# roeiherz/CanonicalSg2Im

Hardware: AMD Instinct MI355X
Metric: 256x256 images/sec/node (G+D step) (higher is better)
Workload: dtype f32; 1 GPU; BASELINE config C3: COCO-shaped AttSPADE 256x256, batch 16/GPU, 1-30 objects/img, ngf=64 ndf=64, --no_vgg_loss --use_img_disc 0; Sg2Layout GCN + SPADE G + 2-scale PatchGAN D + object-crop D, fwd+bwd+Adam; global_batch=16, parallelism=dp1

## Files before the change

### canonicalsg2im_amd/_lib.py

```python
import ctypes
import os

import torch

_HERE = os.path.dirname(os.path.abspath(__file__))
LIB_PATH = os.environ.get("CSG_HIP_LIB") or os.path.join(_HERE, "libcsg_hip.so")

MAX_TAPS = 16
ACT_NONE, ACT_LEAKY, ACT_TANH = 0, 1, 2

c_i32, c_i64, c_f32, c_f64, c_p = ctypes.c_int32, ctypes.c_int64, ctypes.c_float, ctypes.c_double, ctypes.c_void_p


class ConvDesc(ctypes.Structure):
    _fields_ = [
        ("B", c_i32), ("IHp", c_i32), ("IWp", c_i32), ("Cin", c_i32), ("x_cs", c_i32),
        ("IHv", c_i32), ("IWv", c_i32), ("in_up", c_i32),
        ("OHg", c_i32), ("OWg", c_i32), ("OHf", c_i32), ("OWf", c_i32), ("os", c_i32), ("ooy", c_i32), ("oox", c_i32),
        ("Cout", c_i32), ("y_cs", c_i32),
        ("istride", c_i32), ("ntaps", c_i32), ("wtaps", c_i32),
        ("tap_dy", c_i32 * MAX_TAPS), ("tap_dx", c_i32 * MAX_TAPS), ("tap_w", c_i32 * MAX_TAPS),
        ("act", c_i32), ("slope", c_f32), ("accumulate", c_i32), ("res_gate", c_i32),
    ]

# ... 68 lines not shown
    "csg_layout_bwd": (c_i32, [c_p, c_i64, c_i64, c_p, c_p, c_p, c_i64, c_i64, c_i64, c_i64, c_i64, c_i64, c_i64,
                               c_i64, c_p, c_i32, c_p, c_p, c_p, c_i64, c_p]),
    "csg_layout_bwd_masks": (c_i32, [c_p, c_i64, c_i64, c_p, c_p, c_i64, c_i64, c_i64, c_i64, c_i64, c_i64, c_i64, c_i64,
                                     c_p, c_p, c_i32, c_p]),
    "csg_layout_mass": (c_i32, [c_p, c_p, c_p, c_p, c_i64, c_i64, c_i64, c_i64, c_i64, c_i64, c_p, c_p]),
    "csg_layout_paint": (c_i32, [c_p, c_p, c_p, c_i64, c_p, c_i64, c_i64, c_i64, c_i64, c_i64, c_i64, c_i64, c_p, c_i64,
                                 c_i64, c_p]),
    "csg_conv_fwd_workspace": (c_i64, [ctypes.POINTER(ConvDesc)]),
    "csg_conv_fwd": (c_i32, [ctypes.POINTER(ConvDesc), c_p, c_p, c_p, c_p, c_p, c_p, c_i64, c_p]),
    "csg_conv_bwd_weight_workspace": (c_i64, [ctypes.POINTER(ConvDesc)]),
    "csg_conv_bwd_weight": (c_i32, [ctypes.POINTER(ConvDesc), c_p, c_p, c_p, c_p, c_p, c_i64, c_p]),
    "csg_wino_pack_bytes": (c_i64, [c_i64, c_i64]),
    "csg_wino_pack_weights": (c_i32, [c_p, c_i64, c_i64, c_i64, c_i64, c_i64, c_i64, c_i32, c_p, c_p, c_p]),
    "csg_conv_fwd_multi_workspace": (c_i64, [ctypes.POINTER(ConvDesc), c_i32]),
    "csg_conv_fwd_multi": (c_i32, [ctypes.POINTER(ConvDesc), c_i32, c_p, c_p, c_p, c_p, c_p, c_p, c_i64, c_p]),
    "csg_gemm_supported": (c_i32, [ctypes.POINTER(GemmDesc)]),
    "csg_gemm_nt": (c_i32, [ctypes.POINTER(GemmDesc), c_p, c_p, c_p, c_p, c_p, c_p]),
    "csg_gemm_tn_workspace": (c_i64, [c_i64, c_i64, c_i64]),
    "csg_gemm_tn": (c_i32, [c_i64, c_i64, c_i64, c_p, c_i64, c_p, c_i64, c_p, c_p, c_p, c_i64, c_p]),
    "csg_conv_few_supported": (c_i32, [ctypes.POINTER(FewDesc)]),
    "csg_conv_few_fwd_workspace": (c_i64, [ctypes.POINTER(FewDesc)]),
    "csg_conv_few_fwd": (c_i32, [ctypes.POINTER(FewDesc), c_p, c_p, c_p, c_p, c_p, c_i64, c_p]),
    "csg_conv_few_bwd_data": (c_i32, [ctypes.POINTER(FewDesc), c_p, c_p, c_p, c_p]),
    "csg_conv_few_bwd_weight_workspace": (c_i64, [ctypes.POINTER(FewDesc)]),
    "csg_conv_few_bwd_weight": (c_i32, [ctypes.POINTER(FewDesc), c_p, c_p, c_p, c_p, c_p, c_i64, c_p]),
    "csg_wino_conv_workspace": (c_i64, [ctypes.POINTER(WinoDesc)]),
    "csg_wino_conv": (c_i32, [ctypes.POINTER(WinoDesc), c_p, c_p, c_p, c_p, c_p, c_f32, c_p, c_p, c_i64, c_p]),
    "csg_wino_bwd_weight_workspace": (c_i64, [ctypes.POINTER(WinoDesc)]),
    "csg_wino_bwd_weight": (c_i32, [ctypes.POINTER(WinoDesc), c_p, c_p, c_p, c_p, c_p, c_i64, c_p]),
    "csg_wino4_bwd_weight_workspace": (c_i64, [ctypes.POINTER(WinoDesc)]),
    "csg_wino4_bwd_weight": (c_i32, [ctypes.POINTER(WinoDesc), c_p, c_p, c_p, c_p, c_p, c_i64, c_p]),
    "csg_wino4_supported": (c_i32, [ctypes.POINTER(WinoDesc)]),
    "csg_wino4_persistent": (c_i32, [c_i32]),
    "csg_wino_pack_weights_multi": (c_i32, [ctypes.POINTER(WinoPackItem), c_i32, c_p]),
    "csg_wino4_pack_bytes": (c_i64, [c_i64, c_i64]),
    "csg_wino4_pack_weights": (c_i32, [c_p, c_i64, c_i64, c_i64, c_i64, c_i64, c_i64, c_i32, c_p, c_p, c_p]),
    "csg_wino4_conv_workspace": (c_i64, [ctypes.POINTER(WinoDesc)]),
    "csg_wino4_conv": (c_i32, [ctypes.POINTER(WinoDesc), c_p, c_p, c_p, c_p, c_p, c_f32, c_p, c_p, c_i64, c_p]),
    "csg_wino4_conv_part": (c_i32, [ctypes.POINTER(WinoDesc), c_p, c_p, c_i64, c_i64, c_p, c_p, c_p, c_i64, c_p, c_p, c_f32,
                                    c_p, c_p]),
    "csg_wino4_conv_spade_supported": (c_i32, [ctypes.POINTER(WinoDesc)]),
    "csg_wino4_conv_spade": (c_i32, [ctypes.POINTER(WinoDesc), c_p, c_p, c_p, c_p, c_p, c_i64, c_p, c_p, c_f32, c_p, c_p]),
    "csg_wino34_supported": (c_i32, [ctypes.POINTER(WinoDesc), c_i32]),
    "csg_wino34_pack_weights": (c_i32, [c_p, c_i64, c_i64, c_i64, c_i64, c_i64, c_i64, c_i32, c_p, c_p, c_p]),
    "csg_wino34_conv_workspace": (c_i64, [ctypes.POINTER(WinoDesc), c_i32]),
    "csg_wino34_conv": (c_i32, [ctypes.POINTER(WinoDesc), c_i32, c_p, c_p, c_p, c_p, c_p, c_f32, c_p, c_p, c_i64, c_p]),
    "csg_act_bwd": (c_i32, [c_p, c_p, c_i64, c_i32, c_f32, c_p, c_p]),
    "csg_colsum": (c_i32, [c_p, c_i64, c_i64, c_i64, c_p, c_p, c_i64, c_p]),
    "csg_norm_stats": (c_i32, [c_p, c_i64, c_i64, c_i64, c_p, c_p, c_i64, c_p]),
    "csg_norm_finalize": (c_i32, [c_p, c_i64, c_i64, c_f64, c_f32, c_i32, c_p, c_p, c_p, c_p, c_f32, c_p]),
    "csg_norm_stats_finalize": (c_i32, [c_p, c_i64, c_i64, c_i64, c_p, c_i64, c_f64, c_f32, c_p, c_p, c_p, c_p, c_p, c_p, c_f32,
                                        c_p]),
    "csg_norm_apply_fwd": (c_i32, [c_p, c_p, c_p, c_p, c_f32, c_i64, c_i64, c_i64, c_p, c_p, c_f32, c_p, c_p]),
    "csg_norm_eval_stats_multi": (c_i32, [ctypes.POINTER(NormEvalItem), c_i32, c_f32, c_p, c_p]),
    "csg_deprocess_u8_workspace": (c_i64, [c_i64]),
    "csg_deprocess_u8": (c_i32, [c_p, c_i64, c_i64, c_i64, c_i64, ctypes.POINTER(c_f32), ctypes.POINTER(c_f32), c_i32, c_p, c_p,
                                 c_i64, c_p]),
    "csg_preprocess_workspace": (c_i64, [c_p, c_i64, c_i64]),
    "csg_preprocess": (c_i32, [c_p, c_i64, c_p, c_p, c_i64, c_i64, c_i64, ctypes.POINTER(c_f32), ctypes.POINTER(c_f32), c_p, c_p,
                               c_p, c_i64, c_p]),
    "csg_preprocess_px_workspace": (c_i64, [c_p, c_i64, c_i64]),
    "csg_preprocess_px": (c_i32, [c_p, c_i64, c_p, c_p, c_i64, c_i64, c_i64, ctypes.POINTER(c_f32), ctypes.POINTER(c_f32), c_p,
                                  c_p, c_p, c_i64, c_p]),
    "csg_clevr_boxes": (c_i32, [c_p, c_p, c_i64, c_p, c_p, c_p, c_p, c_i64, c_i64, c_p, c_p]),
    "csg_vg_rows": (c_i32, [c_p, c_p, c_p, c_p, c_p, c_p, c_i64, c_i64, c_i64, c_p, c_p, c_p]),
    "csg_draw_boxes_u8": (c_i32, [c_p, c_p, c_p, c_i64, c_i64, c_i64, c_i64, c_i64, c_i64, c_p, c_i64, c_i32, c_p, c_p]),
# ... 108 lines not shown
```

### canonicalsg2im_amd/csrc/wino4.hip

```cpp
#include <stddef.h>
#include <stdlib.h>

#include <type_traits>

#include "csg_buffer.h"
#include "csg_common.h"
#include "csg_pack.h"
#include "csg_reduce.h"

using namespace csg;

typedef __attribute__((ext_vector_type(16))) float f32x16;
typedef const volatile __attribute__((address_space(3))) csg_f32x2* w4_lds_cv2;

#define W4_TW 8
#define W4_TH 4
#define W4_CQ 9
#define W4_PS 8
#define W4_RSE 36
#define W4_NLD 2
#define W4_THREADS 768
#define W4_RBUF (6 * 2 * 32 * W4_RSE)

struct Wino4Params {
// ... 258 lines not shown
          bl2[r] = w4_out_row(2 * half + r, lo) + csg_f32x2{bbv.x, bbv.y};
          bh2[r] = w4_out_row(2 * half + r, hi) + csg_f32x2{bbv.z, bbv.w};
        }
      }
      const float4 mm = *(const float4*)(p.mod_mean + n), mr = *(const float4*)(p.mod_invstd + n);
      const int64_t rowstride = (int64_t)p.Wo * p.y_cs;
      const int64_t pix0 = ((int64_t)img * p.Ho + oy + 2 * half) * p.Wo + ox;
      const int64_t off = pix0 * p.y_cs + n;
      float4 mx[2];
#pragma unroll
      for (int r = 0; r < 2; ++r) mx[r] = *(const float4*)(xin + off + r * rowstride);
#pragma unroll
      for (int r = 0; r < 2; ++r) {
        const csg_f32x2 gl = gl2[r], gh = gh2[r], bl = bl2[r], bh = bh2[r];
        const float gs[4] = {gl.x, gl.y, gh.x, gh.y}, vv[4] = {bl.x, bl.y, bh.x, bh.y};
        const float xs[4] = {mx[r].x, mx[r].y, mx[r].z, mx[r].w};
        const float ms[4] = {mm.x, mm.y, mm.z, mm.w}, rs[4] = {mr.x, mr.y, mr.z, mr.w};
        float out[4];
#pragma unroll
        for (int e = 0; e < 4; ++e) {
          const float xh = (xs[e] - ms[e]) * rs[e];
          float o = xh * (1.f + gs[e]) + vv[e];
          if (p.mod_slope != 1.0f) o = o > 0.f ? o : o * p.mod_slope;
          out[e] = o;
        }
        if (gout != nullptr)
          *(float4*)(gout + (pix0 + (int64_t)r * p.Wo) * p.g_cs + n) = make_float4(gs[0], gs[1], gs[2], gs[3]);
        *(float4*)(y + off + r * rowstride) = make_float4(out[0], out[1], out[2], out[3]);
      }
    }
  }
}

template <int NB>
__device__ __forceinline__ void w4_epilogue(f32x16 (&acc)[6], const Wino4Params& p, float* rbase, int tid, int wave, int grp,
                                            int j, int h, int nt32, int img, int X0, int Y0, const float* __restrict__ bias,
                                            const float* __restrict__ res, const float* __restrict__ gate,
                                            float* __restrict__ y) {
  float* rbuf = rbase + grp * (W4_RBUF / 2 * NB);
  const int tig = tid - grp * (W4_THREADS / 2);
  const bool plain = p.act == CSG_ACT_NONE && res == nullptr && gate == nullptr;
  if (NB == 2) __syncthreads();
  csg_f32x2 rr[NB == 1 ? 4 : 1][8];
  if (NB == 1) {
#pragma unroll
    for (int ge = 0; ge < 8; ++ge) {
#define W4_M(K) csg_f32x2{acc[K][2 * ge], acc[K][2 * ge + 1]}
      const csg_f32x2 m0 = W4_M(0), m1 = W4_M(1), m2 = W4_M(2), m3 = W4_M(3), m4 = W4_M(4), m5 = W4_M(5);
#undef W4_M
      rr[0][ge] = ((m0 + m1) + (m2 + m3)) + m4;
      rr[NB == 1 ? 1 : 0][ge] = w4_pfma(-2.0f, m4, w4_pfma(0.5f, m3, m1 - m2));
      rr[NB == 1 ? 2 : 0][ge] = w4_pfma(4.0f, m4, w4_pfma(0.25f, m3, m1 + m2));
      rr[NB == 1 ? 3 : 0][ge] = w4_pfma(-8.0f, m4, w4_pfma(0.125f, m3, m1 - m2)) + m5;
    }
#pragma unroll
    for (int b = 0; b < (NB == 1 ? 4 : 1); ++b)
#pragma unroll
      for (int ge = 0; ge < 8; ++ge) asm volatile("" : "+v"(rr[b][ge]));
  }
#pragma unroll
  for (int round = 0; round < 4 / NB; ++round) {
#pragma unroll
    for (int g = 0; g < 4; ++g) {
      csg_f32x2 r0[2], r1[2];
#pragma unroll
      for (int e = 0; e < 2; ++e) {
        if (NB == 1) {
          r0[e] = rr[NB == 1 ? round : 0][2 * g + e];
          continue;
        }
#define W4_M(K) csg_f32x2{acc[K][4 * g + 2 * e], acc[K][4 * g + 2 * e + 1]}
        const csg_f32x2 m0 = W4_M(0), m1 = W4_M(1), m2 = W4_M(2), m3 = W4_M(3), m4 = W4_M(4), m5 = W4_M(5);
#undef W4_M
        const int b0 = NB * round;
        if (b0 == 0) r0[e] = ((m0 + m1) + (m2 + m3)) + m4;
        if (b0 == 2) r0[e] = w4_pfma(4.0f, m4, w4_pfma(0.25f, m3, m1 + m2));
        if (b0 == 0) r1[e] = w4_pfma(-2.0f, m4, w4_pfma(0.5f, m3, m1 - m2));
        if (b0 == 2) r1[e] = w4_pfma(-8.0f, m4, w4_pfma(0.125f, m3, m1 - m2)) + m5;
      }
      const int ch = 8 * g + 4 * h;
      *(float4*)(rbuf + ((wave * NB + 0) * 32 + j) * W4_RSE + ch) = make_float4(r0[0].x, r0[0].y, r0[1].x, r0[1].y);
      if (NB == 2)
        *(float4*)(rbuf + ((wave * NB + 1) * 32 + j) * W4_RSE + ch) = make_float4(r1[0].x, r1[0].y, r1[1].x, r1[1].y);
    }
    __syncthreads();
    if (NB == 1 && p.mod == 2)
      w4_store_joint<NB>(p, rbase, tid, round, nt32 - grp * p.gb_off, img, X0, Y0, bias, res, const_cast<float*>(gate), y);
    else if (p.mod)
      w4_store_columns<2, NB>(p, rbuf, tig, round, nt32, img, X0, Y0, bias, res, gate, y);
    else if (plain)
      w4_store_columns<0, NB>(p, rbuf, tig, round, nt32, img, X0, Y0, bias, res, gate, y);
    else
      w4_store_columns<1, NB>(p, rbuf, tig, round, nt32, img, X0, Y0, bias, res, gate, y);
    if (round + 1 < 4 / NB) __syncthreads();
  }
}

__device__ __forceinline__ void w3_epilogue(f32x16 (&acc)[6], const Wino4Params& p, float* smem, int tid, int wave, int grp,
                                            int j, int h, int nt32, int img, int X0, int Y0, const float* __restrict__ bias,
                                            const float* __restrict__ res, const float* __restrict__ gate,
                                            float* __restrict__ y) {
  float* rbuf = smem + grp * W4_RBUF;
  const int tig = tid - grp * (W4_THREADS / 2);
  __syncthreads();
#pragma unroll
  for (int round = 0; round < 2; ++round) {
#pragma unroll
    for (int g = 0; g < 4; ++g) {
      csg_f32x2 r0[2], r1[2];
#pragma unroll
      for (int e = 0; e < 2; ++e) {
#define W4_M(K) csg_f32x2{acc[K][4 * g + 2 * e], acc[K][4 * g + 2 * e + 1]}
        const csg_f32x2 m0 = W4_M(0), m1 = W4_M(1), m2 = W4_M(2), m3 = W4_M(3), m4 = W4_M(4), m5 = W4_M(5);
#undef W4_M
        if (round == 0) {
          r0[e] = ((m0 + m1) + (m2 + m3)) + m4;
          r1[e] = w4_pfma(-2.0f, m4, w4_pfma(0.5f, m3, m1 - m2));
        } else {
          r0[e] = w4_pfma(4.0f, m4, w4_pfma(0.25f, m3, m1 + m2)) + m5;
// ... 60 lines not shown
            vv[0] *= gv.x > 0.f ? 1.f : p.gate_slope; vv[1] *= gv.y > 0.f ? 1.f : p.gate_slope;
            vv[2] *= gv.z > 0.f ? 1.f : p.gate_slope; vv[3] *= gv.w > 0.f ? 1.f : p.gate_slope;
          }
          *(float4*)(y + off) = make_float4(vv[0], vv[1], vv[2], vv[3]);
        }
      }
    }
    if (round == 0) __syncthreads();
  }
}

#define W4_VBUF (36 * 2 * 32 * 4)
template <int T>
struct W4Geo {
  static constexpr int R = T * W4_TH + 6 - T;
  static constexpr int C = T * W4_TW + 6 - T;
  static constexpr int RS = T == 4 ? 288 : 256;
  static constexpr int BUFW = R * RS + 8 + 16;
  static constexpr int V0 = 2 * BUFW;
  static constexpr int OFFTAB = (2 * BUFW + 2 * W4_VBUF) > 2 * W4_RBUF ? (2 * BUFW + 2 * W4_VBUF) : 2 * W4_RBUF;
  static_assert((T * RS) % 64 == 0 && R * C * 2 <= W4_NLD * W4_THREADS && (C + T - 1) / T <= W4_CQ && BUFW < 65536, "staging geometry");
};
#define W4V_RAW0 0
struct W4KernArgs {
  Wino4Params p;
  const float* x;
  const float4* up;
  const float* bias;
  const float* res;
  const float* gate;
  float* y;
};
typedef const __attribute__((address_space(4))) W4KernArgs* w4_kernargs_ptr;
template <int T, bool P>
__global__ __launch_bounds__(W4_THREADS, 3) void k_wino4_conv_v(Wino4Params p, const float* __restrict__ x,
                                                                 const float4* __restrict__ up,
                                                                 const float* __restrict__ bias,
                                                                 const float* __restrict__ res,
                                                                 const float* __restrict__ gate, float* __restrict__ y) {
  typedef W4Geo<T> Geo;
  constexpr int W4_RS = Geo::RS, W4_BUFW = Geo::BUFW, W4V_V0 = Geo::V0, W4V_OFFTAB = Geo::OFFTAB;
  static_assert(!P || T == 4, "the persistent form serves F(4x4,3x3)");
  extern __shared__ __attribute__((aligned(16))) float smem[];
  const int tid = threadIdx.x, lane = tid & 63;
  const int wave12 = __builtin_amdgcn_readfirstlane(tid >> 6);
  const int grp = wave12 >= 6 ? 1 : 0;
  const int wave = wave12 - 6 * grp;

  int nb, img, X0, Y0, split = 0;
  auto decode = [&](int item) {
    if (!P) {
      split = item % p.ksplit;
      item /= p.ksplit;
    }
    nb = item % p.nblocks;
    item /= p.nblocks;
    const int bx = item % p.tbx;
    item /= p.tbx;
    const int by = item % p.tby;
    img = item / p.tby;
    X0 = bx * T * W4_TW;
    Y0 = by * T * W4_TH;
  };
  int v = 0, v_hi = 0, v_step = 1;
  if (P) {
    const int q = p.nitems >> 3, r = p.nitems & 7, xcd = blockIdx.x & 7;
    const int v_lo = xcd < r ? xcd * (q + 1) : r * (q + 1) + (xcd - r) * q;
    v_hi = v_lo + q + (xcd < r ? 1 : 0);
    v_step = gridDim.x >> 3;
    v = v_lo + (blockIdx.x >> 3);
    if (v >= v_hi) return;
    decode(v);
  } else {
    decode(w4_xcd_remap(blockIdx.x, gridDim.x));
  }
// ... 22 lines not shown
          goff[i] = (unsigned)(((img * p.H + iy) * p.W + ix) * p.x_cs + c4 * 4) * 4u;
      }
      loffp |= (unsigned)lo << (16 * i);
    }
    *(uint4*)tab = make_uint4(goff[0], goff[1], loffp, 0u);
  };
  fill_plan(W4_TAB(0), true);
  const int s_begin = split * p.sps, s_end = min(p.nstage, s_begin + p.sps);
  csg_f32x4 st[W4_NLD];
  auto load_stage = [&](int s) {
    const bool over = P && s >= s_end;
    const uint2 go = *(const uint2*)W4_TAB(over ? tsel ^ 1 : tsel);
    if (over) s -= s_end;
    st[0] = csg_buf_load_x4(rsX, (int)go.x, s * (W4_PS * 4), 0);
    st[1] = csg_buf_load_x4(rsX, (int)go.y, s * (W4_PS * 4), 0);
  };
  auto store_stage = [&](float* base) {
    const unsigned lp = s_tab[2];
#pragma unroll
    for (int i = 0; i < W4_NLD; ++i) {
      const unsigned lo = (i & 1) ? (lp >> 16) : (lp & 0xffffu);
      float* dst = base + lo;
      *(float2*)dst = make_float2(st[i].x, st[i].y);
      *(float2*)(dst + 2) = make_float2(st[i].z, st[i].w);
    }
  };

  const int j = lane & 31, h = lane >> 5;
  const int tx = j & (W4_TW - 1), ty = j >> 3;
  const int rb = wave == 0 ? 0 : 1;
  const float* p0 = smem + W4V_RAW0 + (T * ty + rb) * W4_RS + 2 * ty + tx * W4_PS + 4 * grp + 2 * h;
  float* pv = smem + W4V_V0 + (((wave * 6) * 2 + h) * 32 + j) * 4;

  int nt32 = p.gb_off ? nb + grp * p.gb_off : nb * 2 + grp;
  auto u_tile = [&]() { return ((wave * 6) * p.NT32 + nt32 + p.nt_off) * p.Q8 * 1024; };
  const unsigned ulane = nt32 + p.nt_off < p.NT32 || P ? (unsigned)lane * 16u : CSG_OOB_OFF;
  int ubase = u_tile(), ubase_nxt = ubase;
  const int ustride = p.NT32 * p.Q8 * 1024;
  csg_f32x4 ur[3];
  auto load_ur = [&](int slot, int nu, int s) {
    const bool over = P && s >= s_end;
    const int qq = over ? 0 : min(s, p.Q8 - 1);
    ur[slot] = csg_buf_load_x4(rsU, (int)ulane, (over ? ubase_nxt : ubase) + nu * ustride + qq * 1024, 0);
  };

  f32x16 acc[6];

  auto produce_xi = [&](auto xi_tag, int rbufsel, int vbufsel) {
    constexpr int XI = decltype(xi_tag)::value;
    constexpr int RBC = XI == 0 ? 0 : 1;
    constexpr int O2 = 2 * W4_RS + (T == 3 ? 2 * RBC : 0), O3 = 3 * W4_RS + (T == 3 ? 2 : 2 * RBC);
    csg_f32x2 t[6];
#pragma unroll
    for (int c = 0; c < 6; ++c) {
      const int co = rbufsel * W4_BUFW + ((c % T) * W4_CQ + (c / T)) * W4_PS;
      const csg_f32x2 e0 = *(w4_lds_cv2)(p0 + co);
      const csg_f32x2 e1 = *(w4_lds_cv2)(p0 + co + W4_RS);
      const csg_f32x2 e2 = *(w4_lds_cv2)(p0 + co + O2);
      const csg_f32x2 e3 = *(w4_lds_cv2)(p0 + co + O3);
      if (XI == 0 || XI == 5) {
        const csg_f32x2 e4 = *(w4_lds_cv2)(p0 + co + 4 * W4_RS + 2);
        t[c] = w4_pfma(1.5f, e3 - e1, w4_pfma(-2.0f, e2, e0 + e4));
      } else if (XI == 1) {
        t[c] = w4_pfma(2.5f, e2, w4_pfma(0.5f, e1, e3 - e0));
      } else if (XI == 2) {
        t[c] = w4_pfma(0.5f, e2, w4_pfma(-2.5f, e1, e3 + e0));
      } else if (XI == 3) {
        t[c] = w4_pfma(2.0f, e2 - e0, e3 - e1);
      } else {
        t[c] = w4_pfma(-0.5f, e2 - e0, e3 - e1);
      }
    }
    csg_f32x2 v[6];
    {
      const csg_f32x2 s42 = t[4] - t[2], s31 = t[3] - t[1];
      v[0] = w4_pfma(1.5f, s31, w4_pfma(-2.0f, t[2], t[0] + t[4]));
      v[1] = w4_pfma(2.5f, t[3], w4_pfma(0.5f, t[2], t[4] - t[1]));
      v[2] = w4_pfma(0.5f, t[3], w4_pfma(-2.5f, t[2], t[4] + t[1]));
      v[3] = w4_pfma(2.0f, s31, s42);
      v[4] = w4_pfma(-0.5f, s31, s42);
      v[5] = w4_pfma(1.5f, s42, w4_pfma(-2.0f, t[3], t[1] + t[5]));
    }
    int goff2 = 2 * grp;
    if (P) {
      int z;
      asm volatile("s_mov_b32 %0, 0" : "=s"(z));
      goff2 += z;
    }
#pragma unroll
    for (int nu = 0; nu < 6; ++nu)
      *(csg_f32x2*)(pv + vbufsel * W4_VBUF + nu * 256 + goff2) = v[nu];
  };
  auto produce = [&](int rbufsel, int vbufsel) {
    switch (wave) {
      case 0: produce_xi(std::integral_constant<int, 0>(), rbufsel, vbufsel); break;
      case 1: produce_xi(std::integral_constant<int, 1>(), rbufsel, vbufsel); break;
      case 2: produce_xi(std::integral_constant<int, 2>(), rbufsel, vbufsel); break;
      case 3: produce_xi(std::integral_constant<int, 3>(), rbufsel, vbufsel); break;
      case 4: produce_xi(std::integral_constant<int, 4>(), rbufsel, vbufsel); break;
      default: produce_xi(std::integral_constant<int, 5>(), rbufsel, vbufsel); break;
    }
  };
  auto consume = [&](auto lo_tag, auto hi_tag, int vbufsel, int s) {
#pragma unroll
    for (int nu = decltype(lo_tag)::value; nu < decltype(hi_tag)::value; ++nu) {
      const float4 v = *(const float4*)(pv + vbufsel * W4_VBUF + nu * 256);
      const int slot = nu % 3;
      acc[nu] = __builtin_amdgcn_mfma_f32_32x32x2f32(ur[slot].x, v.x, acc[nu], 0, 0, 0);
      acc[nu] = __builtin_amdgcn_mfma_f32_32x32x2f32(ur[slot].y, v.y, acc[nu], 0, 0, 0);
      acc[nu] = __builtin_amdgcn_mfma_f32_32x32x2f32(ur[slot].z, v.z, acc[nu], 0, 0, 0);
      acc[nu] = __builtin_amdgcn_mfma_f32_32x32x2f32(ur[slot].w, v.w, acc[nu], 0, 0, 0);
      if (nu < 3) load_ur(slot, nu + 3, s); else load_ur(slot, nu - 3, s + 1);
    }
  };
  constexpr int SPLIT = 3;
  auto stage = [&](int s, auto par_tag) {
    constexpr int par = decltype(par_tag)::value;
    typedef std::integral_constant<int, 0> I0;
    typedef std::integral_constant<int, SPLIT> IS;
    typedef std::integral_constant<int, 6> I6;
    consume(I0(), IS(), par, s);
    __builtin_amdgcn_sched_barrier(0);
    if (s + 1 < s_end) produce(par ^ 1, par ^ 1);
    __builtin_amdgcn_sched_barrier(0);
    consume(IS(), I6(), par, s);
    store_stage(smem + W4V_RAW0 + par * W4_BUFW);
    __syncthreads();
    load_stage(s + 3);
  };

  y += (long long)split * p.slab;
  {
    const uint2 go = *(const uint2*)W4_TAB(0);
    const csg_f32x4 a0 = csg_buf_load_x4(rsX, (int)go.x, s_begin * (W4_PS * 4), 0);
    const csg_f32x4 a1 = csg_buf_load_x4(rsX, (int)go.y, s_begin * (W4_PS * 4), 0);
    load_stage(s_begin + 1);
#pragma unroll
    for (int nu = 0; nu < 3; ++nu) load_ur(nu, nu, s_begin);
    const csg_f32x4 b0 = st[0], b1 = st[1];
    st[0] = a0;
    st[1] = a1;
    store_stage(smem + W4V_RAW0);
    __syncthreads();
    st[0] = b0;
    st[1] = b1;
    produce(0, 0);
    store_stage(smem + W4V_RAW0 + W4_BUFW);
    __syncthreads();
    load_stage(s_begin + 2);
  }
  for (;;) {
#pragma unroll
    for (int nu = 0; nu < 6; ++nu)
#pragma unroll
      for (int e = 0; e < 16; ++e) acc[nu][e] = 0.f;
    bool more = false;
    int item_n = 0;
    int nb_n = nb, img_n = img, X0_n = X0, Y0_n = Y0;
    if (P) {
      const int nb_c = nb, img_c = img, X0_c = X0, Y0_c = Y0;
      more = v + v_step < v_hi;
      item_n = more ? v + v_step : v;
      if (more) decode(item_n);
      fill_plan(W4_TAB(tsel ^ 1), more);
      nt32 = p.gb_off ? nb + grp * p.gb_off : nb * 2 + grp;
      ubase_nxt = u_tile();
      nb_n = nb; img_n = img; X0_n = X0; Y0_n = Y0;
      nb = nb_c; img = img_c; X0 = X0_c; Y0 = Y0_c;
      nt32 = p.gb_off ? nb + grp * p.gb_off : nb * 2 + grp;
    }
    int s = s_begin;
    for (; s + 1 < s_end; s += 2) {
      stage(s, std::integral_constant<int, 0>());
      stage(s + 1, std::integral_constant<int, 1>());
    }
    if (s < s_end) stage(s, std::integral_constant<int, 0>());
    if (T == 4 && P) {
      int tid_o = (int)(s_tab - (unsigned*)(smem + W4V_OFFTAB)) >> 2;
      asm volatile("" : "+v"(tid_o));
      w4_kernargs_ptr ka = (w4_kernargs_ptr)__builtin_amdgcn_kernarg_segment_ptr();
      asm volatile("" : "+s"(ka));
      Wino4Params pe = p;
#define W4_F(f) pe.f = ka->p.f;
      W4_F(Cout) W4_F(y_cs) W4_F(Ho) W4_F(Wo) W4_F(act) W4_F(slope) W4_F(gate_slope) W4_F(mod) W4_F(g_cs) W4_F(gb_off) W4_F(mod_slope)
      W4_F(mod_mean) W4_F(mod_invstd)
#undef W4_F
      w4_epilogue<1>(acc, pe, smem + W4V_V0, tid_o, wave, grp, tid_o & 31, (tid_o >> 5) & 1, nt32, img, X0, Y0, ka->bias,
                     ka->res, ka->gate, ka->y);
    } else if (T == 4) {
      w4_epilogue<2>(acc, p, smem, tid, wave, grp, j, h, nt32, img, X0, Y0, bias, res, gate, y);
    } else {
      w3_epilogue(acc, p, smem, tid, wave, grp, j, h, nt32, img, X0, Y0, bias, res, gate, y);
    }
    if (!P || !more) break;
    v = item_n;
    nb = nb_n; img = img_n; X0 = X0_n; Y0 = Y0_n;
    nt32 = p.gb_off ? nb + grp * p.gb_off : nb * 2 + grp;
    ubase = ubase_nxt;
    tsel ^= 1;
    __syncthreads();
    produce(0, 0);
    __syncthreads();
  }
#undef W4_TAB
}

static int w4_plan(const csg_wino_desc* d, int T, int pad, Wino4Params& p, size_t& shm, const char* who) {
  CSG_REQUIRE(d != nullptr, CSG_E_BADSHAPE, "%s: null descriptor", who);
  CSG_REQUIRE(d->B > 0 && d->H > 0 && d->W > 0 && d->Cin > 0 && d->Cout > 0, CSG_E_BADSHAPE, "%s: non-positive dimension", who);
  if (T == 4)
    CSG_REQUIRE(d->H % 4 == 0 && d->W % 4 == 0 && d->W >= 32 && d->H >= 16, CSG_E_UNSUPPORTED,
                "%s: F(4x4,3x3) needs H=%d, W=%d multiples of 4, W >= 32, H >= 16", who, d->H, d->W);
  else
    CSG_REQUIRE((pad == 1 || pad == 2) && d->H + 2 * pad >= 4 && d->W + 2 * pad >= 4, CSG_E_UNSUPPORTED,
                "%s: F(3x3,4x4) serves pad 1 or 2 (got %d) on maps of at least 4 - 2 pad pixels", who, pad);
  const int Ho = T == 4 ? d->H : d->H + 2 * pad - 3, Wo = T == 4 ? d->W : d->W + 2 * pad - 3;
  CSG_REQUIRE(d->Cin % 8 == 0 && d->x_cs % 4 == 0 && d->x_cs >= d->Cin && d->Cout % 4 == 0 && d->y_cs % 4 == 0 &&
                  d->y_cs >= d->Cout,
              CSG_E_UNSUPPORTED, "%s: Cin must be a multiple of 8, the other channel counts and strides of 4", who);
  CSG_REQUIRE((int64_t)d->B * (d->H + 1) * (d->W + 1) * (int64_t)(d->x_cs > d->y_cs ? d->x_cs : d->y_cs) * 4 < CSG_MAX_RECORDS,
              CSG_E_UNSUPPORTED, "%s: tensor too large for 32-bit byte offsets", who);
  CSG_REQUIRE((int64_t)36 * ((d->Cout + 31) / 32) * ((d->Cin + 7) / 8) * 1024 < CSG_MAX_RECORDS, CSG_E_UNSUPPORTED,
              "%s: packed weights too large for 32-bit byte offsets", who);
  p.B = d->B; p.H = d->H; p.W = d->W; p.Cin = d->Cin; p.x_cs = d->x_cs; p.Cout = d->Cout; p.y_cs = d->y_cs;
  p.Ho = Ho; p.Wo = Wo; p.pad = pad;
  p.tbx = (Wo + T * W4_TW - 1) / (T * W4_TW);
  p.tby = (Ho + T * W4_TH - 1) / (T * W4_TH);
  p.nblocks = (d->Cout + 63) / 64;
  p.NT32 = (d->Cout + 31) / 32;
  p.Q8 = (d->Cin + 7) / 8;
  p.act = d->act; p.slope = d->slope; p.gate_slope = 0.f;
  p.nt_off = 0; p.mod = 0; p.g_cs = 0; p.gb_off = 0; p.mod_slope = 1.f; p.mod_mean = nullptr; p.mod_invstd = nullptr;
  p.nstage = d->Cin / W4_PS;
  p.ksplit = 1;
  p.sps = p.nstage;
  p.slab = (long long)d->B * Ho * Wo * d->y_cs;
  p.nitems = 0;
  shm = (size_t)((T == 4 ? W4Geo<4>::OFFTAB : W4Geo<3>::OFFTAB) + W4_THREADS * 4) * 4;
  return CSG_OK;
}

template <int T, bool P>
static int w4_set_lds_limit(const char* who) {
  static DeviceOnce attr_once;
  int dev = 0;
  (void)hipGetDevice(&dev);
  if (attr_once.pending(dev)) {
    hipError_t e = hipFuncSetAttribute((const void*)k_wino4_conv_v<T, P>, hipFuncAttributeMaxDynamicSharedMemorySize,
                                       (P ? 160 : 128) * 1024);
    CSG_REQUIRE(e == hipSuccess, CSG_E_LAUNCH, "%s: cannot raise the dynamic LDS limit: %s", who, hipGetErrorString(e));
    attr_once.mark(dev);
  }
  return CSG_OK;
}

static std::atomic<int> w4_persist_on{-1};
static int w4_persistent_blocks(const Wino4Params& p, int64_t items) {
  static std::atomic<int> cus[32];
  int on = w4_persist_on.load(std::memory_order_relaxed);
  if (on < 0) {
    on = getenv("CSG_WINO4_PERSIST") ? atoi(getenv("CSG_WINO4_PERSIST")) : 1;
    int expect = -1;
    w4_persist_on.compare_exchange_strong(expect, on);
    on = w4_persist_on.load(std::memory_order_relaxed);
  }
  int dev = 0;
  (void)hipGetDevice(&dev);
  if (!on || dev < 0) return 0;
  int ncu = dev < 32 ? cus[dev].load(std::memory_order_relaxed) : 0;
  if (ncu == 0) {
    if (hipDeviceGetAttribute(&ncu, hipDeviceAttributeMultiprocessorCount, dev) != hipSuccess || ncu < 8) ncu = -1;
    if (dev < 32) cus[dev].store(ncu, std::memory_order_relaxed);
  }
  const int g = ncu > 0 ? (ncu & ~7) : 0;
  if (g == 0 || p.ksplit != 1 || (p.nstage & 1) || p.nstage < 4 || (p.gb_off == 0 && (p.Cout & 63)) || items < 2 * (int64_t)g) return 0;
  return g;
}

template <int T>
static int w4_launch(Wino4Params& p, size_t shm, int kid, double flops, const float* x, const float* packed,
                     const float* bias, const float* residual, const float* gate, float* y, float* workspace,
                     float* y_final, hipStream_t s, const char* who) {
  CSG_REQUIRE(shm <= 128 * 1024, CSG_E_UNSUPPORTED, "%s: %zu bytes of LDS", who, shm);
  const int64_t grid = (int64_t)p.B * p.tby * p.tbx * p.nblocks * p.ksplit;
  CSG_REQUIRE(grid < (1ll << 31), CSG_E_UNSUPPORTED, "%s: grid too large", who);
  p.nitems = (int)grid;
  const int pblocks = T == 4 ? w4_persistent_blocks(p, grid) : 0;
  int rc = pblocks ? w4_set_lds_limit<4, true>(who) : w4_set_lds_limit<T, false>(who);
  if (rc) return rc;
  ProfScope ps(kid, flops, s);
  if (pblocks)
    CSG_LAUNCH((k_wino4_conv_v<4, true>), dim3((unsigned)pblocks), dim3(W4_THREADS), shm + W4_THREADS * 16, s, p, x,
               (const float4*)packed, bias, residual, gate, y);
  else
    CSG_LAUNCH((k_wino4_conv_v<T, false>), dim3((unsigned)grid), dim3(W4_THREADS), shm, s, p, x, (const float4*)packed, bias,
               residual, gate, y);
  rc = check_launch(who);
  if (rc == CSG_OK && p.ksplit > 1) {
    launch_slab_reduce(workspace, p.slab, y_final, nullptr, 0, nullptr, p.ksplit, s);
    rc = check_launch("csg_wino4_conv(slab sum)");
  }
  return rc;
}

static void w4_split_plan(Wino4Params& p, bool plain) {
  if (!plain || p.y_cs != p.Cout) return;
  const int64_t blocks = (int64_t)p.B * p.tby * p.tbx * p.nblocks;
  if (blocks >= 384 || p.nstage < 32) return;
  int ks = (int)((512 + blocks - 1) / blocks);
  if (ks > p.nstage / 16) ks = p.nstage / 16;
  if (ks < 2) return;
  p.sps = (p.nstage + ks - 1) / ks;
  p.ksplit = (p.nstage + p.sps - 1) / p.sps;
}

extern "C" {

int32_t csg_wino4_supported(const csg_wino_desc* d) {
  static const int on = getenv("CSG_WINO4") ? atoi(getenv("CSG_WINO4")) : 1;
  if (!on || d == nullptr) return 0;
  return (d->H % 4 == 0 && d->W % 4 == 0 && d->W >= 32 && d->H >= 16 && d->Cin % 8 == 0 && d->Cout % 4 == 0) ? 1 : 0;
}

int csg_wino4_pack_multi_launch(const PackMulti* pm, int blocks, double bytes, hipStream_t s) {
// ... 27 lines not shown
      CSG_REQUIRE(it.w != nullptr && it.packed != nullptr && it.Cout > 0 && it.Cin > 0 && ((uintptr_t)it.packed % 16) == 0,
                  CSG_E_BADSHAPE, "csg_wino_pack_weights_multi: item %d: bad arguments", i);
      const int64_t N = it.backward_data ? it.Cin : it.Cout, K = it.backward_data ? it.Cout : it.Cin;
      const int64_t s_n = it.backward_data ? it.s_i : it.s_o, s_k = it.backward_data ? it.s_o : it.s_i;
      const int64_t span = (it.Cout - 1) * it.s_o + (it.Cin - 1) * it.s_i + 2 * it.s_h + 2 * it.s_w;
      CSG_REQUIRE(span < (1ll << 31) && s_n >= 0 && s_k >= 0 && it.s_h >= 0 && it.s_w >= 0, CSG_E_UNSUPPORTED,
                  "csg_wino_pack_weights_multi: item %d: weight too large for 32-bit element offsets", i);
      const int NT32 = (int)cdiv(N, 32), Q8 = (int)cdiv(K, 8);
      const int nb = (int)cdiv(Q8, 4) * NT32;
      if (cnt == CSG_PACK_MULTI || blocks + nb > (1 << 20)) {
        const int rc = flush();
        if (rc) return rc;
      }
      PackMultiItem& d = pm.it[cnt++];
      d.w = it.w; d.up = (float4*)it.packed;
      d.s_n = (int)s_n; d.s_k = (int)s_k; d.s_h = (int)it.s_h; d.s_w = (int)it.s_w;
      d.flip = it.backward_data ? 1 : 0; d.N = (int)N; d.K = (int)K; d.NT32 = NT32; d.Q8 = Q8;
      d.start = blocks;
      blocks += nb;
      bytes += (double)it.Cout * it.Cin * 9 * 4 + (double)(variant == 4 ? 36 : 16) * NT32 * Q8 * 64 * 16;
    }
    const int rc = flush();
    if (rc) return rc;
  }
  return CSG_OK;
}

int32_t csg_wino4_persistent(int32_t on) {
  const int prev = w4_persist_on;
  if (on >= 0) w4_persist_on = on != 0;
  return prev;
}

int64_t csg_wino4_pack_bytes(int64_t N, int64_t K) {
  if (N <= 0 || K <= 0) return -1;
  return (int64_t)36 * cdiv(N, 32) * cdiv(K, 8) * 64 * 16;
}

int csg_wino4_pack_weights(const float* w, int64_t s_o, int64_t s_i, int64_t s_h, int64_t s_w, int64_t Cout, int64_t Cin,
                           int32_t backward_data, const float* sigma, float* packed, void* stream) {
  CSG_REQUIRE(w != nullptr && packed != nullptr && Cout > 0 && Cin > 0, CSG_E_BADSHAPE, "csg_wino4_pack_weights: bad arguments");
  CSG_REQUIRE(((uintptr_t)packed % 16) == 0, CSG_E_UNSUPPORTED, "csg_wino4_pack_weights: packed must be 16-byte aligned");
  const int64_t N = backward_data ? Cin : Cout, K = backward_data ? Cout : Cin;
  const int64_t s_n = backward_data ? s_i : s_o, s_k = backward_data ? s_o : s_i;
  const int NT32 = (int)cdiv(N, 32), Q8 = (int)cdiv(K, 8);
  const int64_t total = (int64_t)36 * NT32 * Q8 * 64;
  hipStream_t s = (hipStream_t)stream;
  ProfScope ps(K_WINO_PACK, (double)Cout * Cin * 9 * 4 + (double)total * 16, s);
  CSG_LAUNCH(k_wino4_pack<3>, dim3((unsigned)cdiv(Q8, 4), (unsigned)NT32), dim3(256), 0, s, w, s_n, s_k, s_h, s_w,
                     backward_data ? 1 : 0, (int)N, (int)K, sigma, NT32, Q8, (float4*)packed);
  return check_launch("csg_wino4_pack_weights");
}

int csg_wino34_pack_weights(const float* w, int64_t s_o, int64_t s_i, int64_t s_h, int64_t s_w, int64_t Cout, int64_t Cin,
                            int32_t backward_data, const float* sigma, float* packed, void* stream) {
  CSG_REQUIRE(w != nullptr && packed != nullptr && Cout > 0 && Cin > 0, CSG_E_BADSHAPE, "csg_wino34_pack_weights: bad arguments");
  CSG_REQUIRE(((uintptr_t)packed % 16) == 0, CSG_E_UNSUPPORTED, "csg_wino34_pack_weights: packed must be 16-byte aligned");
  const int64_t N = backward_data ? Cin : Cout, K = backward_data ? Cout : Cin;
  const int64_t s_n = backward_data ? s_i : s_o, s_k = backward_data ? s_o : s_i;
  const int NT32 = (int)cdiv(N, 32), Q8 = (int)cdiv(K, 8);
  const int64_t total = (int64_t)36 * NT32 * Q8 * 64;
  hipStream_t s = (hipStream_t)stream;
  ProfScope ps(K_WINO_PACK, (double)Cout * Cin * 16 * 4 + (double)total * 16, s);
  CSG_LAUNCH(k_wino4_pack<4>, dim3((unsigned)cdiv(Q8, 4), (unsigned)NT32), dim3(256), 0, s, w, s_n, s_k, s_h, s_w,
                     backward_data ? 1 : 0, (int)N, (int)K, sigma, NT32, Q8, (float4*)packed);
  return check_launch("csg_wino34_pack_weights");
// ... 153 lines not shown
```

### include/csg_hip.h

```cpp
#ifndef CSG_HIP_H
#define CSG_HIP_H

#include <stdint.h>

#ifdef __cplusplus
extern "C" {
#endif

#define CSG_OK 0
#define CSG_E_BADSHAPE (-1)
#define CSG_E_UNSUPPORTED (-2)
#define CSG_E_LAUNCH (-3)
#define CSG_E_WORKSPACE (-4)

#define CSG_ACT_NONE 0
#define CSG_ACT_LEAKY 1
#define CSG_ACT_TANH 2

#define CSG_MAX_TAPS 16

int csg_version(void);
const char* csg_last_error(void);

int csg_prof_enable(int mode);
// ... 79 lines not shown
typedef struct csg_wino_desc {
  int32_t B, H, W;
  int32_t Cin, x_cs;
  int32_t Cout, y_cs;
  int32_t act;
  float slope;
} csg_wino_desc;
int64_t csg_wino_pack_bytes(int64_t N, int64_t K);
int csg_wino_pack_weights(const float* w, int64_t s_o, int64_t s_i, int64_t s_h, int64_t s_w, int64_t Cout, int64_t Cin,
                          int32_t backward_data, const float* sigma, float* packed, void* stream);
int64_t csg_wino_conv_workspace(const csg_wino_desc* d);
int csg_wino_conv(const csg_wino_desc* d, const float* x, const float* packed, const float* bias,
                  const float* residual, const float* gate, float gate_slope, float* y, float* workspace,
                  int64_t workspace_bytes, void* stream);
int64_t csg_wino_bwd_weight_workspace(const csg_wino_desc* d);
int csg_wino_bwd_weight(const csg_wino_desc* d, const float* x, const float* dy, float* dw, float* db, float* workspace,
                        int64_t workspace_bytes, void* stream);

int64_t csg_wino4_bwd_weight_workspace(const csg_wino_desc* d);
int csg_wino4_bwd_weight(const csg_wino_desc* d, const float* x, const float* dy, float* dw, float* db, float* workspace,
                         int64_t workspace_bytes, void* stream);

int32_t csg_wino4_supported(const csg_wino_desc* d);
typedef struct csg_wino_pack_item {
  const float* w;
  int64_t s_o, s_i, s_h, s_w;
  int64_t Cout, Cin;
  int32_t backward_data;
  int32_t variant;
  float* packed;
} csg_wino_pack_item;
int csg_wino_pack_weights_multi(const csg_wino_pack_item* items, int32_t n, void* stream);
int32_t csg_wino4_persistent(int32_t on);
int64_t csg_wino4_pack_bytes(int64_t N, int64_t K);
int csg_wino4_pack_weights(const float* w, int64_t s_o, int64_t s_i, int64_t s_h, int64_t s_w, int64_t Cout, int64_t Cin,
                           int32_t backward_data, const float* sigma, float* packed, void* stream);
int64_t csg_wino4_conv_workspace(const csg_wino_desc* d);
int csg_wino4_conv(const csg_wino_desc* d, const float* x, const float* packed, const float* bias,
                   const float* residual, const float* gate, float gate_slope, float* y, float* workspace,
                   int64_t workspace_bytes, void* stream);

int csg_wino4_conv_part(const csg_wino_desc* d, const float* x, const float* packed, int64_t tile_off, int64_t tiles_total,
                        const float* bias, const float* mod_x, const float* mod_gamma, int64_t gamma_cs,
                        const float* mod_mean, const float* mod_invstd, float mod_slope, float* y, void* stream);

int32_t csg_wino4_conv_spade_supported(const csg_wino_desc* d);
int csg_wino4_conv_spade(const csg_wino_desc* d, const float* x, const float* packed, const float* bias, const float* mod_x,
                         float* gamma_out, int64_t gamma_cs, const float* mod_mean, const float* mod_invstd, float mod_slope,
                         float* y, void* stream);

int32_t csg_wino34_supported(const csg_wino_desc* d, int32_t pad);
int csg_wino34_pack_weights(const float* w, int64_t s_o, int64_t s_i, int64_t s_h, int64_t s_w, int64_t Cout, int64_t Cin,
                            int32_t backward_data, const float* sigma, float* packed, void* stream);
int64_t csg_wino34_conv_workspace(const csg_wino_desc* d, int32_t pad);
int csg_wino34_conv(const csg_wino_desc* d, int32_t pad, const float* x, const float* packed, const float* bias,
                    const float* residual, const float* gate, float gate_slope, float* y, float* workspace,
                    int64_t workspace_bytes, void* stream);

typedef struct csg_few_desc {
  int32_t B, IH, IW;
  int32_t Cin, x_cs;
  int32_t KH, KW, pad;
  int32_t cout_real;
  int32_t act;
  float slope;
  int32_t in_act;
// ... 197 lines not shown
```

Before: 216.1 img/s.

## Add 32-output-channel Winograd F(4x4,3x3) kernel splitting transform positions across wave groups

Adds a specialised Winograd kernel for convolutions with at most 32 output channels. Instead of the two wave groups each owning a different 32-channel block, where one group would sit idle, each group handles half of the six transform positions for the same channel block. The second group's accumulators are then handed to the first through LDS before the output transform and epilogue. This aims to stop wasting half the block on narrow convolutions such as the final RGB or early layers, at the cost of extra LDS traffic, extra barriers and a larger dynamic LDS request.

```diff
diff --git a/canonicalsg2im_amd/_lib.py b/canonicalsg2im_amd/_lib.py
--- a/canonicalsg2im_amd/_lib.py
+++ b/canonicalsg2im_amd/_lib.py
@@ -124,6 +124,8 @@
     "csg_wino4_bwd_weight": (c_i32, [ctypes.POINTER(WinoDesc), c_p, c_p, c_p, c_p, c_p, c_i64, c_p]),
     "csg_wino4_supported": (c_i32, [ctypes.POINTER(WinoDesc)]),
     "csg_wino4_persistent": (c_i32, [c_i32]),
+    "csg_wino4_n32": (c_i32, [c_i32]),
+    "csg_wino4_n32_launches": (c_i64, []),
     "csg_wino_pack_weights_multi": (c_i32, [ctypes.POINTER(WinoPackItem), c_i32, c_p]),
     "csg_wino4_pack_bytes": (c_i64, [c_i64, c_i64]),
     "csg_wino4_pack_weights": (c_i32, [c_p, c_i64, c_i64, c_i64, c_i64, c_i64, c_i64, c_i32, c_p, c_p, c_p]),
diff --git a/canonicalsg2im_amd/csrc/wino4.hip b/canonicalsg2im_amd/csrc/wino4.hip
--- a/canonicalsg2im_amd/csrc/wino4.hip
+++ b/canonicalsg2im_amd/csrc/wino4.hip
@@ -314,21 +314,28 @@
   }
 }
 
-template <int NB>
+template <int NB, bool ONE = false>
 __device__ __forceinline__ void w4_epilogue(f32x16 (&acc)[6], const Wino4Params& p, float* rbase, int tid, int wave, int grp,
                                             int j, int h, int nt32, int img, int X0, int Y0, const float* __restrict__ bias,
                                             const float* __restrict__ res, const float* __restrict__ gate,
-                                            float* __restrict__ y) {
+                                            float* __restrict__ y, const float* hx = nullptr) {
   float* rbuf = rbase + grp * (W4_RBUF / 2 * NB);
   const int tig = tid - grp * (W4_THREADS / 2);
   const bool plain = p.act == CSG_ACT_NONE && res == nullptr && gate == nullptr;
   if (NB == 2) __syncthreads();
   csg_f32x2 rr[NB == 1 ? 4 : 1][8];
-  if (NB == 1) {
+  if (NB == 1 && !(ONE && grp)) {
 #pragma unroll
     for (int ge = 0; ge < 8; ++ge) {
 #define W4_M(K) csg_f32x2{acc[K][2 * ge], acc[K][2 * ge + 1]}
-      const csg_f32x2 m0 = W4_M(0), m1 = W4_M(1), m2 = W4_M(2), m3 = W4_M(3), m4 = W4_M(4), m5 = W4_M(5);
+      const csg_f32x2 m0 = W4_M(0), m1 = W4_M(1), m2 = W4_M(2);
+      csg_f32x2 m3, m4, m5;
+      if (ONE) {
+        const csg_f32x2* hq = (const csg_f32x2*)(hx + (ge >> 1) * 256) + (ge & 1);
+        m3 = hq[0]; m4 = hq[4 * 128]; m5 = hq[8 * 128];
+      } else {
+        m3 = W4_M(3); m4 = W4_M(4); m5 = W4_M(5);
+      }
 #undef W4_M
       rr[0][ge] = ((m0 + m1) + (m2 + m3)) + m4;
       rr[NB == 1 ? 1 : 0][ge] = w4_pfma(-2.0f, m4, w4_pfma(0.5f, m3, m1 - m2));
@@ -340,10 +347,12 @@
 #pragma unroll
       for (int ge = 0; ge < 8; ++ge) asm volatile("" : "+v"(rr[b][ge]));
   }
+  if (NB == 1 && ONE) __syncthreads();
 #pragma unroll
   for (int round = 0; round < 4 / NB; ++round) {
 #pragma unroll
     for (int g = 0; g < 4; ++g) {
+      if (ONE && grp) break;
       csg_f32x2 r0[2], r1[2];
 #pragma unroll
       for (int e = 0; e < 2; ++e) {
@@ -366,7 +375,9 @@
         *(float4*)(rbuf + ((wave * NB + 1) * 32 + j) * W4_RSE + ch) = make_float4(r1[0].x, r1[0].y, r1[1].x, r1[1].y);
     }
     __syncthreads();
-    if (NB == 1 && p.mod == 2)
+    if (ONE && grp)
+      ;
+    else if (NB == 1 && p.mod == 2)
       w4_store_joint<NB>(p, rbase, tid, round, nt32 - grp * p.gb_off, img, X0, Y0, bias, res, const_cast<float*>(gate), y);
     else if (p.mod)
       w4_store_columns<2, NB>(p, rbuf, tig, round, nt32, img, X0, Y0, bias, res, gate, y);
@@ -493,15 +504,16 @@
   float* y;
 };
 typedef const __attribute__((address_space(4))) W4KernArgs* w4_kernargs_ptr;
-template <int T, bool P>
-__global__ __launch_bounds__(W4_THREADS, 3) void k_wino4_conv_v(Wino4Params p, const float* __restrict__ x,
-                                                                 const float4* __restrict__ up,
-                                                                 const float* __restrict__ bias,
-                                                                 const float* __restrict__ res,
-                                                                 const float* __restrict__ gate, float* __restrict__ y) {
+template <int T, bool P, bool N32>
+__device__ __forceinline__ void w4_conv_body(const Wino4Params& p, const float* __restrict__ x,
+                                             const float4* __restrict__ up, const float* __restrict__ bias,
+                                             const float* __restrict__ res, const float* __restrict__ gate,
+                                             float* __restrict__ y) {
   typedef W4Geo<T> Geo;
   constexpr int W4_RS = Geo::RS, W4_BUFW = Geo::BUFW, W4V_V0 = Geo::V0, W4V_OFFTAB = Geo::OFFTAB;
   static_assert(!P || T == 4, "the persistent form serves F(4x4,3x3)");
+  static_assert(!N32 || T == 4, "the 32-channel form serves F(4x4,3x3)");
+  static_assert(!N32 || 6 * 12 * 64 * 4 <= (P ? 2 * W4_VBUF : Geo::OFFTAB), "the accumulator hand-over does not fit");
   extern __shared__ __attribute__((aligned(16))) float smem[];
   const int tid = threadIdx.x, lane = tid & 63;
   const int wave12 = __builtin_amdgcn_readfirstlane(tid >> 6);
@@ -590,8 +602,10 @@
   const float* p0 = smem + W4V_RAW0 + (T * ty + rb) * W4_RS + 2 * ty + tx * W4_PS + 4 * grp + 2 * h;
   float* pv = smem + W4V_V0 + (((wave * 6) * 2 + h) * 32 + j) * 4;
 
-  int nt32 = p.gb_off ? nb + grp * p.gb_off : nb * 2 + grp;
-  auto u_tile = [&]() { return ((wave * 6) * p.NT32 + nt32 + p.nt_off) * p.Q8 * 1024; };
+  auto u_tile_of = [&](int b) { return N32 ? b * 2 : p.gb_off ? b + grp * p.gb_off : b * 2 + grp; };
+  int nt32 = u_tile_of(nb);
+  const int nu0 = N32 ? 3 * grp : 0;
+  auto u_tile = [&]() { return ((wave * 6 + nu0) * p.NT32 + nt32 + p.nt_off) * p.Q8 * 1024; };
   const unsigned ulane = nt32 + p.nt_off < p.NT32 || P ? (unsigned)lane * 16u : CSG_OOB_OFF;
   int ubase = u_tile(), ubase_nxt = ubase;
   const int ustride = p.NT32 * p.Q8 * 1024;
@@ -603,6 +617,8 @@
   };
 
   f32x16 acc[6];
+  constexpr int NPOS = N32 ? 3 : 6;
+  const float* pvc = N32 ? pv + nu0 * 256 : pv;
 
   auto produce_xi = [&](auto xi_tag, int rbufsel, int vbufsel) {
     constexpr int XI = decltype(xi_tag)::value;
@@ -662,21 +678,21 @@
   auto consume = [&](auto lo_tag, auto hi_tag, int vbufsel, int s) {
 #pragma unroll
     for (int nu = decltype(lo_tag)::value; nu < decltype(hi_tag)::value; ++nu) {
-      const float4 v = *(const float4*)(pv + vbufsel * W4_VBUF + nu * 256);
+      const float4 v = *(const float4*)(pvc + vbufsel * W4_VBUF + nu * 256);
       const int slot = nu % 3;
       acc[nu] = __builtin_amdgcn_mfma_f32_32x32x2f32(ur[slot].x, v.x, acc[nu], 0, 0, 0);
       acc[nu] = __builtin_amdgcn_mfma_f32_32x32x2f32(ur[slot].y, v.y, acc[nu], 0, 0, 0);
       acc[nu] = __builtin_amdgcn_mfma_f32_32x32x2f32(ur[slot].z, v.z, acc[nu], 0, 0, 0);
       acc[nu] = __builtin_amdgcn_mfma_f32_32x32x2f32(ur[slot].w, v.w, acc[nu], 0, 0, 0);
-      if (nu < 3) load_ur(slot, nu + 3, s); else load_ur(slot, nu - 3, s + 1);
+      if (N32) load_ur(slot, nu, s + 1); else if (nu < 3) load_ur(slot, nu + 3, s); else load_ur(slot, nu - 3, s + 1);
     }
   };
-  constexpr int SPLIT = 3;
+  constexpr int SPLIT = N32 ? 2 : 3;
   auto stage = [&](int s, auto par_tag) {
     constexpr int par = decltype(par_tag)::value;
     typedef std::integral_constant<int, 0> I0;
     typedef std::integral_constant<int, SPLIT> IS;
-    typedef std::integral_constant<int, 6> I6;
+    typedef std::integral_constant<int, NPOS> I6;
     consume(I0(), IS(), par, s);
     __builtin_amdgcn_sched_barrier(0);
     if (s + 1 < s_end) produce(par ^ 1, par ^ 1);
@@ -709,7 +725,7 @@
   }
   for (;;) {
 #pragma unroll
-    for (int nu = 0; nu < 6; ++nu)
+    for (int nu = 0; nu < NPOS; ++nu)
 #pragma unroll
       for (int e = 0; e < 16; ++e) acc[nu][e] = 0.f;
     bool more = false;
@@ -721,11 +737,11 @@
       item_n = more ? v + v_step : v;
       if (more) decode(item_n);
       fill_plan(W4_TAB(tsel ^ 1), more);
-      nt32 = p.gb_off ? nb + grp * p.gb_off : nb * 2 + grp;
+      nt32 = u_tile_of(nb);
       ubase_nxt = u_tile();
       nb_n = nb; img_n = img; X0_n = X0; Y0_n = Y0;
       nb = nb_c; img = img_c; X0 = X0_c; Y0 = Y0_c;
-      nt32 = p.gb_off ? nb + grp * p.gb_off : nb * 2 + grp;
+      nt32 = u_tile_of(nb);
     }
     int s = s_begin;
     for (; s + 1 < s_end; s += 2) {
@@ -743,8 +759,44 @@
       W4_F(Cout) W4_F(y_cs) W4_F(Ho) W4_F(Wo) W4_F(act) W4_F(slope) W4_F(gate_slope) W4_F(mod) W4_F(g_cs) W4_F(gb_off) W4_F(mod_slope)
       W4_F(mod_mean) W4_F(mod_invstd)
 #undef W4_F
-      w4_epilogue<1>(acc, pe, smem + W4V_V0, tid_o, wave, grp, tid_o & 31, (tid_o >> 5) & 1, nt32, img, X0, Y0, ka->bias,
-                     ka->res, ka->gate, ka->y);
+      if (N32) {
+        float* hx = smem + W4V_V0 + (wave * 12 * 64 + (tid_o & 63)) * 4;
+        __syncthreads();
+        if (grp) {
+#pragma unroll
+          for (int i = 0; i < 3; ++i)
+#pragma unroll
+            for (int q = 0; q < 4; ++q)
+              *(float4*)(hx + (i * 4 + q) * 256) = make_float4(acc[i][4 * q], acc[i][4 * q + 1], acc[i][4 * q + 2], acc[i][4 * q + 3]);
+        }
+        __syncthreads();
+        w4_epilogue<1, true>(acc, pe, smem + W4V_V0, tid_o, wave, grp, tid_o & 31, (tid_o >> 5) & 1, nt32, img, X0, Y0,
+                             ka->bias, ka->res, ka->gate, ka->y, hx);
+      } else {
+        w4_epilogue<1>(acc, pe, smem + W4V_V0, tid_o, wave, grp, tid_o & 31, (tid_o >> 5) & 1, nt32, img, X0, Y0, ka->bias,
+                       ka->res, ka->gate, ka->y);
+      }
+    } else if (T == 4 && N32) {
+      float* hx = smem + (wave * 12 * 64 + lane) * 4;
+      __syncthreads();
+      if (grp) {
+#pragma unroll
+        for (int i = 0; i < 3; ++i)
+#pragma unroll
+          for (int q = 0; q < 4; ++q)
+            *(float4*)(hx + (i * 4 + q) * 256) = make_float4(acc[i][4 * q], acc[i][4 * q + 1], acc[i][4 * q + 2], acc[i][4 * q + 3]);
+      }
+      __syncthreads();
+      if (!grp) {
+#pragma unroll
+        for (int i = 0; i < 3; ++i)
+#pragma unroll
+          for (int q = 0; q < 4; ++q) {
+            const float4 m = *(const float4*)(hx + (i * 4 + q) * 256);
+            acc[3 + i][4 * q] = m.x; acc[3 + i][4 * q + 1] = m.y; acc[3 + i][4 * q + 2] = m.z; acc[3 + i][4 * q + 3] = m.w;
+          }
+      }
+      w4_epilogue<2, true>(acc, p, smem, tid, wave, grp, j, h, nt32, img, X0, Y0, bias, res, gate, y);
     } else if (T == 4) {
       w4_epilogue<2>(acc, p, smem, tid, wave, grp, j, h, nt32, img, X0, Y0, bias, res, gate, y);
     } else {
@@ -753,7 +805,7 @@
     if (!P || !more) break;
     v = item_n;
     nb = nb_n; img = img_n; X0 = X0_n; Y0 = Y0_n;
-    nt32 = p.gb_off ? nb + grp * p.gb_off : nb * 2 + grp;
+    nt32 = u_tile_of(nb);
     ubase = ubase_nxt;
     tsel ^= 1;
     __syncthreads();
@@ -761,6 +813,24 @@
     __syncthreads();
   }
 #undef W4_TAB
+}
+
+template <int T, bool P>
+__global__ __launch_bounds__(W4_THREADS, 3) void k_wino4_conv_v(Wino4Params p, const float* __restrict__ x,
+                                                                 const float4* __restrict__ up,
+                                                                 const float* __restrict__ bias,
+                                                                 const float* __restrict__ res,
+                                                                 const float* __restrict__ gate, float* __restrict__ y) {
+  w4_conv_body<T, P, false>(p, x, up, bias, res, gate, y);
+}
+
+template <bool P>
+__global__ __launch_bounds__(W4_THREADS, 3) void k_wino4_conv_n32(Wino4Params p, const float* __restrict__ x,
+                                                                   const float4* __restrict__ up,
+                                                                   const float* __restrict__ bias,
+                                                                   const float* __restrict__ res,
+                                                                   const float* __restrict__ gate, float* __restrict__ y) {
+  w4_conv_body<4, P, true>(p, x, up, bias, res, gate, y);
 }
 
 static int w4_plan(const csg_wino_desc* d, int T, int pad, Wino4Params& p, size_t& shm, const char* who) {
@@ -813,7 +883,7 @@
 }
 
 static std::atomic<int> w4_persist_on{-1};
-static int w4_persistent_blocks(const Wino4Params& p, int64_t items) {
+static int w4_persistent_blocks(const Wino4Params& p, int64_t items, bool n32 = false) {
   static std::atomic<int> cus[32];
   int on = w4_persist_on.load(std::memory_order_relaxed);
   if (on < 0) {
@@ -831,8 +901,24 @@
     if (dev < 32) cus[dev].store(ncu, std::memory_order_relaxed);
   }
   const int g = ncu > 0 ? (ncu & ~7) : 0;
-  if (g == 0 || p.ksplit != 1 || (p.nstage & 1) || p.nstage < 4 || (p.gb_off == 0 && (p.Cout & 63)) || items < 2 * (int64_t)g) return 0;
+  if (g == 0 || p.ksplit != 1 || (p.nstage & 1) || p.nstage < 4 || (p.gb_off == 0 && !n32 && (p.Cout & 63)) || items < 2 * (int64_t)g) return 0;
   return g;
+}
+
+static std::atomic<int> w4_n32_on{1};
+static std::atomic<long long> w4_n32_count{0};
+template <bool P>
+static int w4_n32_set_lds_limit(const char* who) {
+  static DeviceOnce attr_once;
+  int dev = 0;
+  (void)hipGetDevice(&dev);
+  if (attr_once.pending(dev)) {
+    hipError_t e = hipFuncSetAttribute((const void*)k_wino4_conv_n32<P>, hipFuncAttributeMaxDynamicSharedMemorySize,
+                                       (P ? 160 : 128) * 1024);
+    CSG_REQUIRE(e == hipSuccess, CSG_E_LAUNCH, "%s: cannot raise the dynamic LDS limit: %s", who, hipGetErrorString(e));
+    attr_once.mark(dev);
+  }
+  return CSG_OK;
 }
 
 template <int T>
@@ -843,11 +929,22 @@
   const int64_t grid = (int64_t)p.B * p.tby * p.tbx * p.nblocks * p.ksplit;
   CSG_REQUIRE(grid < (1ll << 31), CSG_E_UNSUPPORTED, "%s: grid too large", who);
   p.nitems = (int)grid;
-  const int pblocks = T == 4 ? w4_persistent_blocks(p, grid) : 0;
-  int rc = pblocks ? w4_set_lds_limit<4, true>(who) : w4_set_lds_limit<T, false>(who);
+  const bool n32 = T == 4 && p.Cout <= 32 && p.nblocks == 1 && p.ksplit == 1 && p.mod == 0 && p.gb_off == 0 &&
+                   w4_n32_on.load(std::memory_order_relaxed) != 0;
+  const int pblocks = T == 4 ? w4_persistent_blocks(p, grid, n32) : 0;
+  int rc = n32 ? (pblocks ? w4_n32_set_lds_limit<true>(who) : w4_n32_set_lds_limit<false>(who))
+               : pblocks ? w4_set_lds_limit<4, true>(who) : w4_set_lds_limit<T, false>(who);
   if (rc) return rc;
   ProfScope ps(kid, flops, s);
-  if (pblocks)
+  if (n32) {
+    if (pblocks)
+      CSG_LAUNCH(k_wino4_conv_n32<true>, dim3((unsigned)pblocks), dim3(W4_THREADS), shm + W4_THREADS * 16, s, p, x,
+                 (const float4*)packed, bias, residual, gate, y);
+    else
+      CSG_LAUNCH(k_wino4_conv_n32<false>, dim3((unsigned)grid), dim3(W4_THREADS), shm, s, p, x, (const float4*)packed, bias,
+                 residual, gate, y);
+    w4_n32_count.fetch_add(1, std::memory_order_relaxed);
+  } else if (pblocks)
     CSG_LAUNCH((k_wino4_conv_v<4, true>), dim3((unsigned)pblocks), dim3(W4_THREADS), shm + W4_THREADS * 16, s, p, x,
                (const float4*)packed, bias, residual, gate, y);
   else
@@ -941,6 +1038,14 @@
   return prev;
 }
 
+int32_t csg_wino4_n32(int32_t on) {
+  const int prev = w4_n32_on;
+  if (on >= 0) w4_n32_on = on != 0;
+  return prev;
+}
+
+int64_t csg_wino4_n32_launches(void) { return (int64_t)w4_n32_count.load(std::memory_order_relaxed); }
+
 int64_t csg_wino4_pack_bytes(int64_t N, int64_t K) {
   if (N <= 0 || K <= 0) return -1;
   return (int64_t)36 * cdiv(N, 32) * cdiv(K, 8) * 64 * 16;
diff --git a/include/csg_hip.h b/include/csg_hip.h
--- a/include/csg_hip.h
+++ b/include/csg_hip.h
@@ -135,6 +135,8 @@
 } csg_wino_pack_item;
 int csg_wino_pack_weights_multi(const csg_wino_pack_item* items, int32_t n, void* stream);
 int32_t csg_wino4_persistent(int32_t on);
+int32_t csg_wino4_n32(int32_t on);
+int64_t csg_wino4_n32_launches(void);
 int64_t csg_wino4_pack_bytes(int64_t N, int64_t K);
 int csg_wino4_pack_weights(const float* w, int64_t s_o, int64_t s_i, int64_t s_h, int64_t s_w, int64_t Cout, int64_t Cin,
                            int32_t backward_data, const float* sigma, float* packed, void* stream);
```

Result: no change. 217.0 img/s (median of 6 runs) (+0.4%).
